# DichenZhang1/libultrahdr_dev

Hardware: AMD Instinct MI355X
Metric: MPixels/sec gain-map generate+apply, 4K P010 batch (higher is better)
Workload: dtype u8/u16 in, f32+f64 math, u8/u32 out

## Files before the change

libultrahdr_dev_amd/build.py:

```python
import os
import subprocess
import sys

HERE = os.path.dirname(os.path.abspath(__file__))
CSRC = os.path.join(HERE, "csrc")
ROOT = os.path.dirname(HERE)
LIB = os.path.join(HERE, "libuhdr_hip.so")
SHIM_LIB = os.path.join(HERE, "libultrahdr_shim.so")
COMM_LIB = os.path.join(HERE, "libuhdr_hip_comm.so")

SOURCES = ["uhdr_kernels.hip", "uhdr_capi.hip", "uhdr_jpeg.hip", "uhdr_jpeg_dec.hip", "uhdr_jpeg_hdr.cpp", "uhdr_jpeg_prog.cpp", "uhdr_jpegr.cpp"]
DEPS = SOURCES + ["uhdr_kernels.h", "uhdr_device_math.h", "uhdr_jpeg.h", "uhdr_jpegr.h", os.path.join(ROOT, "include", "uhdr_hip.h")]
COMM_SOURCES = ["uhdr_comm.hip"]
COMM_DEPS = COMM_SOURCES + [os.path.join(ROOT, "include", "uhdr_hip_comm.h")]
SHIM_SOURCES = ["ultrahdr_shim.cpp"]
SHIM_DEPS = SHIM_SOURCES + [os.path.join(ROOT, "include", "uhdr_hip.h"),
                            os.path.join(ROOT, "include", "ultrahdr_hip", "ultrahdr_hip.h")]

HIPCC = os.environ.get("HIPCC", "/opt/rocm/bin/hipcc")
FLAGS = ["--offload-arch=gfx950", "-O3", "-std=c++17", "-fPIC", "-ffp-contract=off",
         "-fno-fast-math", "-Wall", "-Wno-unused-function"]


def _stale(target, deps, base):
    if not os.path.exists(target):
        return True
    t = os.path.getmtime(target)
    for d in deps:
        p = d if os.path.isabs(d) else os.path.join(base, d)
        if os.path.exists(p) and os.path.getmtime(p) > t:
            return True
    return False


def build(force=False, verbose=False):
    if force or _stale(LIB, DEPS, CSRC):
        cmd = [HIPCC] + FLAGS + ["-shared", "-o", LIB] + [os.path.join(CSRC, s) for s in SOURCES]
        if verbose:
            print(" ".join(cmd))
        subprocess.check_call(cmd)
    shim_src = [os.path.join(CSRC, s) for s in SHIM_SOURCES]
    if all(os.path.exists(s) for s in shim_src) and (force or _stale(SHIM_LIB, SHIM_DEPS, CSRC)):
        cmd = ["g++", "-O2", "-std=c++17", "-fPIC", "-shared", "-I" + os.path.join(ROOT, "include"),
               "-o", SHIM_LIB] + shim_src + ["-L" + HERE, "-luhdr_hip", "-Wl,-rpath,$ORIGIN"]
        if verbose:
            print(" ".join(cmd))
        subprocess.check_call(cmd)
    if force or _stale(COMM_LIB, COMM_DEPS, CSRC):
        rocm_lib = os.path.join(os.path.dirname(os.path.dirname(HIPCC)), "lib")
        cmd = [HIPCC] + FLAGS + ["-shared", "-o", COMM_LIB] + [os.path.join(CSRC, s) for s in COMM_SOURCES] + ["-L" + rocm_lib, "-lrccl", "-Wl,-rpath," + rocm_lib]
        if verbose:
            print(" ".join(cmd))
        try:
            subprocess.check_call(cmd)
        except (subprocess.CalledProcessError, OSError) as e:
            print("libuhdr_hip_comm.so skipped (is RCCL installed under %s?): %s" % (rocm_lib, e), file=sys.stderr)
    return LIB


if __name__ == "__main__":
    print(build(force="--force" in sys.argv, verbose=True))
```

libultrahdr_dev_amd/csrc/uhdr_kernels.hip:

```cpp
#include "uhdr_kernels.h"

#include <hip/hip_runtime.h>

#include <algorithm>
#include <cmath>

#include "uhdr_device_math.h"
#include "uhdr_wave_scan.h"

namespace uhdr {

__constant__ float c_idw4[4 * 64];

__constant__ float c_idw4p[64];

hipError_t upload_idw4(const float* tables) {
  float p[64];
  for (int oy = 0; oy < 4; ++oy)
    for (int pr = 0; pr < 2; ++pr)
      for (int k = 0; k < 4; ++k)
        for (int h = 0; h < 2; ++h) p[((oy * 2 + pr) * 4 + k) * 2 + h] = tables[oy * 16 + (2 * pr + h) * 4 + k];
  hipError_t e = hipMemcpyToSymbol(HIP_SYMBOL(c_idw4p), p, sizeof(p));
  if (e != hipSuccess) return e;
  return hipMemcpyToSymbol(HIP_SYMBOL(c_idw4), tables, sizeof(float) * 4 * 64);
// ... 1272 lines not shown
    o.z = (b * factor) / c.display_boost;
  } else {
    r = srgb_inv_oetf_fast(r); g = srgb_inv_oetf_fast(g); b = srgb_inv_oetf_fast(b);
    const float factor = __builtin_amdgcn_exp2f((log_boost * c.display_boost) * c.inv_max_boost);
    o.x = (r * factor) * c.inv_display_boost;
    o.y = (g * factor) * c.inv_display_boost;
    o.z = (b * factor) * c.inv_display_boost;
  }
  return o;
}

template <int FMT, bool EXACT>
__device__ __forceinline__ F3 hdr_oetf(F3 e) {
  if (FMT == 3) {
    if (EXACT) { float ch[3] = {e.x, e.y, e.z}; hlg_oetf_guarded_n<3>(ch); e.x = ch[0]; e.y = ch[1]; e.z = ch[2]; }
    else { e.x = hlg_oetf_fast(e.x); e.y = hlg_oetf_fast(e.y); e.z = hlg_oetf_fast(e.z); }
  } else if (FMT == 2) {
    if (EXACT) { float ch[3] = {e.x, e.y, e.z}; pq_oetf_guarded_n<3>(ch); e.x = ch[0]; e.y = ch[1]; e.z = ch[2]; }
    else { e.x = pq_oetf_est(e.x); e.y = pq_oetf_est(e.y); e.z = pq_oetf_est(e.z); }
  }
  return e;
}

__device__ __forceinline__ float map_to_float(uint32_t v) { return (float)v / 255.0f; }
__device__ __forceinline__ float map_to_float_fast(uint32_t v) { return div_const((float)v, 255.0f, 1.0f / 255.0f); }

__device__ __forceinline__ f2 log2_2(f2 v) { return (f2){__builtin_amdgcn_logf(v.x), __builtin_amdgcn_logf(v.y)}; }
__device__ __forceinline__ f2 exp2_2(f2 v) { return (f2){__builtin_amdgcn_exp2f(v.x), __builtin_amdgcn_exp2f(v.y)}; }
__device__ __forceinline__ f2 sqrt_2(f2 v) { return (f2){__builtin_amdgcn_sqrtf(v.x), __builtin_amdgcn_sqrtf(v.y)}; }
__device__ __forceinline__ f2 rcp_2(f2 v) { return (f2){__builtin_amdgcn_rcpf(v.x), __builtin_amdgcn_rcpf(v.y)}; }
__device__ __forceinline__ f2 sel_le(f2 x, float thr, f2 a, f2 b) {
  return (f2){x.x <= thr ? a.x : b.x, x.y <= thr ? a.y : b.y};
}


__device__ __forceinline__ f2 srgb_eotf2(f2 e) {
  constexpr float kThr = 0.04045f;
  const f2 a = pk_mul_sat(e, splat(1.0f / kThr));
  const f2 lin = pk_fma(a, splat(kThr / 12.92f), splat(-(kThr / 12.92f)));
  const f2 d = pk_add_sat(e, splat(-kThr));
  const f2 x = pk_fma(d, splat(1.0f / 1.055f), splat((kThr + 0.055f) / 1.055f));
  const f2 t = exp2_2(log2_2(x) * splat(0.4f));
  return pk_fma(x * x, t, lin);
}

__device__ __forceinline__ uint32_t tab_offset(float x) {
  typedef __fp16 h2 __attribute__((ext_vector_type(2)));
  const h2 q = __builtin_amdgcn_cvt_pkrtz(x, 0.0f);
  return __builtin_bit_cast(uint32_t, q) & 0x7FF8u;
}
__device__ __forceinline__ uint32_t pow_offset(float x) {
  uint32_t off;
  asm("v_and_b32_sdwa %0, %1, %2 dst_sel:DWORD dst_unused:UNUSED_PAD src0_sel:DWORD src1_sel:WORD_1" : "=v"(off) : "v"(0x0FF8u), "v"(x));
  return off;
}
__device__ __forceinline__ void pow_pair(f2 x, const char* lut, float2& a, float2& b) {
  a = *reinterpret_cast<const float2*>(lut + pow_offset(x.x));
  b = *reinterpret_cast<const float2*>(lut + pow_offset(x.y));
}
template <uint32_t BASE>
__device__ __forceinline__ void tab_pair(f2 x, const char* lut, float2& a, float2& b) {
  typedef __fp16 h2 __attribute__((ext_vector_type(2)));
  const h2 q = __builtin_amdgcn_cvt_pkrtz(x.x, x.y);
  const uint32_t d = __builtin_bit_cast(uint32_t, q);
  uint32_t hi_off;
  asm("v_and_b32_sdwa %0, %1, %2 dst_sel:DWORD dst_unused:UNUSED_PAD src0_sel:DWORD src1_sel:WORD_1" : "=v"(hi_off) : "v"(0x7FF8u), "v"(d));
  a = *reinterpret_cast<const float2*>(lut + BASE + (d & 0x7FF8u));
  b = *reinterpret_cast<const float2*>(lut + BASE + hi_off);
}
template <uint32_t BASE>
__device__ __forceinline__ f2 tab_eval2(f2 x, const char* lut) {
  float2 a, b;
  tab_pair<BASE>(x, lut, a, b);
  f2 o;
  asm("v_fma_f32 %0, %1, %2, %3" : "=v"(o.x) : "v"(a.y), "v"(x.x), "v"(a.x));
  asm("v_fma_f32 %0, %1, %2, %3" : "=v"(o.y) : "v"(b.y), "v"(x.y), "v"(b.x));
  return o;
}
__device__ __forceinline__ uint32_t s2_address(float s, uint32_t slot8) {
  return __builtin_amdgcn_perm(__float_as_uint(s), slot8, 0x0C0C0600u);
}
__device__ __forceinline__ f2 code_eval2(f2 s, uint32_t slot8, const char* lut) {
  const float2 a = *reinterpret_cast<const float2*>(lut + s2_address(s.x, slot8));
  const float2 b = *reinterpret_cast<const float2*>(lut + s2_address(s.y, slot8));
  f2 o;
  asm("v_fma_f32 %0, %1, %2, %3" : "=v"(o.x) : "v"(a.y), "v"(s.x), "v"(a.x));
  asm("v_fma_f32 %0, %1, %2, %3" : "=v"(o.y) : "v"(b.y), "v"(s.y), "v"(b.x));
  return o;
}

template <int FMT, bool MASK> struct ApplyTab {
  static constexpr bool kOetf = !MASK && (FMT == 2 || FMT == 3);
  static constexpr uint32_t kS1Bytes = kOetf ? kTabS1PowBytes : kTabS1Bytes;
  static constexpr uint32_t kS2Base = kS1Bytes;
  static constexpr uint32_t kS2Bytes = kOetf ? kTabS2LdsBytes : 0u;
  static constexpr uint32_t kBytes = kS1Bytes + kS2Bytes;
  static constexpr uint32_t kS1Float = !kOetf ? kTabS1Lin : FMT == 3 ? kTabS1Hlg : kTabS1Pq;
  static constexpr uint32_t kS2Float = FMT == 3 ? kTabS2Hlg : kTabS2Pq;
};

template <int FMT>
__device__ __forceinline__ f2 oetf2_scaled(f2 e) {
  if (FMT == 3) {
    const f2 lo = sqrt_2(e * splat(3.0f * 1023.0f * 1023.0f));
    const f2 hi = pk_fma(log2_2(pk_fma(e, splat(12.0f), splat(-UHDR_HLG_B))),
                         splat(UHDR_HLG_A * 0.693147180559945f * 1023.0f), splat(UHDR_HLG_C * 1023.0f));
    return sel_le(e, 1.0f / 12.0f, lo, hi);
  } else if (FMT == 2) {
    const f2 p = exp2_2(log2_2(e) * splat(UHDR_PQ_M1));
    const f2 q = pk_fma(p, splat(UHDR_PQ_C2), splat(UHDR_PQ_C1)) * rcp_2(pk_fma(p, splat(UHDR_PQ_C3), splat(1.0f)));
    return exp2_2(pk_fma(log2_2(q), splat(UHDR_PQ_M2), splat(9.99859042974533f)));
  } else if (FMT == 4) {
    return e * splat(1023.0f);
  }
  return e;
}

struct PairOut { f2 r, g, b; };

template <bool MASK>
__device__ __forceinline__ uint32_t pack10_scaled(float r, float g, float b) {
  uint32_t ri = (uint32_t)r, gi = (uint32_t)g, bi = (uint32_t)b;
  if (MASK) { ri &= 0x3ffu; gi &= 0x3ffu; bi &= 0x3ffu; }
  uint32_t t;
  asm("v_lshl_or_b32 %0, %1, 10, %2" : "=v"(t) : "v"(gi), "v"(ri));
  asm("v_lshl_or_b32 %0, %1, 20, %2" : "=v"(t) : "v"(bi), "v"(t));
  return t | 0xC0000000u;
}
__device__ __forceinline__ uint32_t pack10_bits(float r, float g, float b) {
  uint32_t t;
  asm("v_lshl_or_b32 %0, %1, 10, %2" : "=v"(t) : "v"(__float_as_uint(g)), "v"(__float_as_uint(r)));
  asm("v_lshl_or_b32 %0, %1, 20, %2" : "=v"(t) : "v"(__float_as_uint(b)), "v"(t));
  return t;
}

template <int K>
__device__ __forceinline__ float cvt_byte(uint32_t w) { return (float)((w >> (8 * K)) & 0xffu); }

struct PairF { f2 c[3]; f2 factor; float2 e[6]; };
struct PairM { f2 s[3]; float2 e[6]; };
struct ChromaRow { f2 crv, ngs, cbu; };
__device__ __forceinline__ ChromaRow chroma_row(uint32_t uu, uint32_t vv) {
  constexpr float kCrS = kP3Cr * k255, kCbS = kP3Cb * k255, kGCbS = kP3GCb * k255, kGCrS = kP3GCr * k255;
  const f2 uf = (f2){cvt_byte<0>(uu), cvt_byte<1>(uu)};
  const f2 vf = (f2){cvt_byte<0>(vv), cvt_byte<1>(vv)};
  ChromaRow o;
  o.crv = pk_fma(vf, splat(kCrS), splat(-128.0f * kCrS));
  o.cbu = pk_fma(uf, splat(kCbS), splat(-128.0f * kCbS));
  o.ngs = pk_fma(uf, splat(-kGCbS), pk_fma(vf, splat(-kGCrS), splat(128.0f * kGCbS + 128.0f * kGCrS)));
  return o;
}
template <int FMT>
__device__ __forceinline__ void apply_cell_piped(const AppConsts& c, void* dst, uint32_t cx, uint32_t cy,
                                                 const uint32_t (&yrow)[4], const uint32_t (&uu)[2], const uint32_t (&vv)[2],
                                                 float m1, float m2, float m3, float m4, uint32_t slot8, const char* lut) {
  typedef ApplyTab<FMT, false> T;
  ChromaRow cr = chroma_row(uu[0], vv[0]);
  const float a255 = c.fast.A255;
  f2 d23 = (f2){m2 - m1, m3 - m1}, d4b = (f2){m4 - m1, __builtin_fmaf(m1, a255, c.fast.B)};
  asm("" : "+v"(d23), "+v"(d4b));
  PairF pf[2];
  PairM pm[2];
  uint32_t px[4];
#pragma unroll
  for (int k = 0; k < 10; ++k) {
    if (k < 8) {
      const int oy = k >> 1, pr = k & 1;
      const f2 w1 = (f2){c.fast.wD[oy][pr][0][0], c.fast.wD[oy][pr][0][1]}, w2 = (f2){c.fast.wD[oy][pr][1][0], c.fast.wD[oy][pr][1][1]};
      const f2 w3 = (f2){c.fast.wD[oy][pr][2][0], c.fast.wD[oy][pr][2][1]};
      if (k == 4) cr = chroma_row(uu[1], vv[1]);
      PairF& f = pf[k & 1];
      const f2 E = pk_fma(bc_lo(d4b), w3, pk_fma(bc_hi(d23), w2, pk_fma(bc_lo(d23), w1, bc_hi(d4b))));
      const f2 yraw = pr ? (f2){cvt_byte<2>(yrow[oy]), cvt_byte<3>(yrow[oy])} : (f2){cvt_byte<0>(yrow[oy]), cvt_byte<1>(yrow[oy])};
      if (pr) {
        f.c[0] = pk_fma_sat_bc<1>(yraw, splat(k255), cr.crv); f.c[1] = pk_fma_sat_bc<1>(yraw, splat(k255), cr.ngs);
        f.c[2] = pk_fma_sat_bc<1>(yraw, splat(k255), cr.cbu);
      } else {
        f.c[0] = pk_fma_sat_bc<0>(yraw, splat(k255), cr.crv); f.c[1] = pk_fma_sat_bc<0>(yraw, splat(k255), cr.ngs);
        f.c[2] = pk_fma_sat_bc<0>(yraw, splat(k255), cr.cbu);
      }
      f.factor = exp2_2(E);
#pragma unroll
      for (int ch = 0; ch < 3; ++ch) pow_pair(f.c[ch], lut, f.e[2 * ch], f.e[2 * ch + 1]);
    }
    __builtin_amdgcn_sched_barrier(0);
    if (k >= 1 && k <= 8) {
      PairF& f = pf[(k - 1) & 1];
      PairM& m = pm[(k - 1) & 1];
#pragma unroll
      for (int ch = 0; ch < 3; ++ch) {
        f2 t;
        asm("v_fma_f32 %0, %1, %2, %3" : "=v"(t.x) : "v"(f.e[2 * ch].y), "v"(f.c[ch].x), "v"(f.e[2 * ch].x));
        asm("v_fma_f32 %0, %1, %2, %3" : "=v"(t.y) : "v"(f.e[2 * ch + 1].y), "v"(f.c[ch].y), "v"(f.e[2 * ch + 1].x));
        m.s[ch] = pk_fma(t, f.factor, splat(2.0f));
      }
#pragma unroll
      for (int ch = 0; ch < 3; ++ch) {
        m.e[2 * ch] = *reinterpret_cast<const float2*>(lut + T::kS2Base + s2_address(m.s[ch].x, slot8));
        m.e[2 * ch + 1] = *reinterpret_cast<const float2*>(lut + T::kS2Base + s2_address(m.s[ch].y, slot8));
      }
    }
    __builtin_amdgcn_sched_barrier(0);
    if (k >= 2) {
      const int q = k - 2, oy = q >> 1, pr = q & 1;
      PairM& m = pm[q & 1];
      float o[6];
#pragma unroll
      for (int ch = 0; ch < 3; ++ch) {
        asm("v_fma_f32 %0, %1, %2, %3" : "=v"(o[2 * ch]) : "v"(m.e[2 * ch].y), "v"(m.s[ch].x), "v"(m.e[2 * ch].x));
        asm("v_fma_f32 %0, %1, %2, %3" : "=v"(o[2 * ch + 1]) : "v"(m.e[2 * ch + 1].y), "v"(m.s[ch].y), "v"(m.e[2 * ch + 1].x));
      }
      px[2 * pr] = pack10_bits(o[0], o[2], o[4]);
      px[2 * pr + 1] = pack10_bits(o[1], o[3], o[5]);
      if (pr) {
        const uint32_t off = ((4u * cy + oy) * c.width + 4u * cx) * 4u;
        st_stream(reinterpret_cast<uint4*>(static_cast<char*>(dst) + off), make_uint4(px[0], px[1], px[2], px[3]));
      }
    }
    __builtin_amdgcn_sched_barrier(0);
  }
}

constexpr uint32_t kXchSecond = 72;
constexpr uint32_t kXchPerWave = 136;
template <int FMT, bool MASK>
__device__ __forceinline__ void apply_cell_piped1(const AppConsts& c, const AppImage& im, uint32_t cx, uint32_t cy,
                                                  const uint32_t (&yrow)[4], const uint32_t (&uu)[2], const uint32_t (&vv)[2],
                                                  float m1, float m2, float m3, float m4, const char* lut, uint4* xch) {
  ChromaRow cr = chroma_row(uu[0], vv[0]);
  const float a255 = c.fast.A255;
  f2 d23 = (f2){m2 - m1, m3 - m1}, d4b = (f2){m4 - m1, __builtin_fmaf(m1, a255, c.fast.B)};
  asm("" : "+v"(d23), "+v"(d4b));
  PairF pf[2];
  PairOut po[2];
  const uint32_t lane = threadIdx.x & 63u;
#pragma unroll
  for (int k = 0; k < 9; ++k) {
    if (k < 8) {
      const int oy = k >> 1, pr = k & 1;
      const f2 w1 = (f2){c.fast.wD[oy][pr][0][0], c.fast.wD[oy][pr][0][1]}, w2 = (f2){c.fast.wD[oy][pr][1][0], c.fast.wD[oy][pr][1][1]};
      const f2 w3 = (f2){c.fast.wD[oy][pr][2][0], c.fast.wD[oy][pr][2][1]};
      if (k == 4) cr = chroma_row(uu[1], vv[1]);
      PairF& f = pf[k & 1];
      const f2 E = pk_fma(bc_lo(d4b), w3, pk_fma(bc_hi(d23), w2, pk_fma(bc_lo(d23), w1, bc_hi(d4b))));
      const f2 yraw = pr ? (f2){cvt_byte<2>(yrow[oy]), cvt_byte<3>(yrow[oy])} : (f2){cvt_byte<0>(yrow[oy]), cvt_byte<1>(yrow[oy])};
      if (pr) {
        f.c[0] = pk_fma_sat_bc<1>(yraw, splat(k255), cr.crv); f.c[1] = pk_fma_sat_bc<1>(yraw, splat(k255), cr.ngs);
        f.c[2] = pk_fma_sat_bc<1>(yraw, splat(k255), cr.cbu);
      } else {
        f.c[0] = pk_fma_sat_bc<0>(yraw, splat(k255), cr.crv); f.c[1] = pk_fma_sat_bc<0>(yraw, splat(k255), cr.ngs);
        f.c[2] = pk_fma_sat_bc<0>(yraw, splat(k255), cr.cbu);
      }
      f.factor = exp2_2(E);
#pragma unroll
      for (int ch = 0; ch < 3; ++ch) tab_pair<0>(f.c[ch], lut, f.e[2 * ch], f.e[2 * ch + 1]);
    }
    __builtin_amdgcn_sched_barrier(0);
    if (k >= 1) {
      const int q = k - 1, oy = q >> 1, pr = q & 1;
      PairF& f = pf[q & 1];
      f2 lin[3];
#pragma unroll
      for (int ch = 0; ch < 3; ++ch) {
        f2 t;
        asm("v_fma_f32 %0, %1, %2, %3" : "=v"(t.x) : "v"(f.e[2 * ch].y), "v"(f.c[ch].x), "v"(f.e[2 * ch].x));
        asm("v_fma_f32 %0, %1, %2, %3" : "=v"(t.y) : "v"(f.e[2 * ch + 1].y), "v"(f.c[ch].y), "v"(f.e[2 * ch + 1].x));
        lin[ch] = oetf2_scaled<FMT>(t * f.factor);
      }
      po[pr].r = lin[0]; po[pr].g = lin[1]; po[pr].b = lin[2];
      if (pr) {
        const uint32_t pix0 = (4u * cy + oy) * c.width + 4u * cx;
        if (FMT == 2 || FMT == 3) {
          uint4 o;
          o.x = pack10_scaled<MASK>(po[0].r.x, po[0].g.x, po[0].b.x); o.y = pack10_scaled<MASK>(po[0].r.y, po[0].g.y, po[0].b.y);
          o.z = pack10_scaled<MASK>(po[1].r.x, po[1].g.x, po[1].b.x); o.w = pack10_scaled<MASK>(po[1].r.y, po[1].g.y, po[1].b.y);
          st_stream(reinterpret_cast<uint4*>(static_cast<uint32_t*>(im.dst) + pix0), o);
        } else if (FMT == 1) {
          const uint2 a = pack_f16_hw(po[0].r.x, po[0].g.x, po[0].b.x), bb = pack_f16_hw(po[0].r.y, po[0].g.y, po[0].b.y);
          const uint2 cc = pack_f16_hw(po[1].r.x, po[1].g.x, po[1].b.x), d = pack_f16_hw(po[1].r.y, po[1].g.y, po[1].b.y);
          if (xch != nullptr) {
            xch[lane] = make_uint4(a.x, a.y, bb.x, bb.y);
            xch[kXchSecond + lane] = make_uint4(cc.x, cc.y, d.x, d.y);
            __builtin_amdgcn_wave_barrier();
            const uint32_t from = (lane & 1u) * kXchSecond + (lane >> 1);
            const uint4 s0 = xch[from], s1 = xch[from + 32u];
            __builtin_amdgcn_wave_barrier();
            uint4* o = reinterpret_cast<uint4*>(static_cast<uint2*>(im.dst) + (uint32_t)__builtin_amdgcn_readfirstlane((int)pix0));
            st_stream(o + lane, s0);
            st_stream(o + 64u + lane, s1);
          } else {
            uint4* o = reinterpret_cast<uint4*>(static_cast<uint2*>(im.dst) + pix0);
            o[0] = make_uint4(a.x, a.y, bb.x, bb.y);
            o[1] = make_uint4(cc.x, cc.y, d.x, d.y);
          }
        } else {
          const size_t plane = (size_t)c.width * c.height;
          uint16_t* base16 = static_cast<uint16_t*>(im.dst);
          const f2 ch[3][2] = {{po[0].r, po[1].r}, {po[0].g, po[1].g}, {po[0].b, po[1].b}};
#pragma unroll
          for (int p = 0; p < 3; ++p) {
            const uint32_t q0 = 0x3ffu & (uint32_t)ch[p][0].x, q1 = 0x3ffu & (uint32_t)ch[p][0].y;
            const uint32_t q2 = 0x3ffu & (uint32_t)ch[p][1].x, q3 = 0x3ffu & (uint32_t)ch[p][1].y;
            st_stream(reinterpret_cast<uint2*>(base16 + p * plane + pix0), make_uint2(q0 | (q1 << 16), q2 | (q3 << 16)));
          }
        }
      }
    }
    __builtin_amdgcn_sched_barrier(0);
  }
}

struct ApplyCellIn { uint32_t yrow[4], uu[2], vv[2], mb[4]; };
__device__ __forceinline__ void apply_load_cell(const AppConsts& c, const AppImage& im, uint32_t cx, uint32_t cy, ApplyCellIn& o) {
  const uint32_t yoff = 4u * cy * im.y_stride + 4u * cx;
#pragma unroll
  for (int r = 0; r < 4; ++r) o.yrow[r] = ld_stream(reinterpret_cast<const uint32_t*>(im.y + (yoff + r * im.y_stride)));
  const uint32_t coff = 2u * cy * im.c_stride + 2u * cx;
#pragma unroll
  for (int r = 0; r < 2; ++r) {
    o.uu[r] = *reinterpret_cast<const uint16_t*>(im.u + (coff + r * im.c_stride));
    o.vv[r] = *reinterpret_cast<const uint16_t*>(im.v + (coff + r * im.c_stride));
  }
  const uint32_t xu = min(cx + 1u, c.map_w - 1u), yu = min(cy + 1u, c.map_h - 1u);
  const uint32_t m0 = cy * c.map_w, m1 = yu * c.map_w;
  o.mb[0] = im.map[m0 + cx]; o.mb[1] = im.map[m1 + cx]; o.mb[2] = im.map[m0 + xu]; o.mb[3] = im.map[m1 + xu];
}

template <int FMT, bool MASK>
__device__ __forceinline__ void apply_cell_edge(const AppConsts& c, const AppImage& im, uint32_t cx, uint32_t cy,
                                                const uint32_t (&yrow)[4], const uint32_t (&uu)[2], const uint32_t (&vv)[2],
                                                float m1, float m2, float m3, float m4, const float* wt ,
                                                uint32_t slot8, const char* lut) {
  typedef ApplyTab<FMT, MASK> T;
  const float a255 = c.fast.A255;
  const float base = __builtin_fmaf(m1, a255, c.fast.B), d2 = m2 - m1, d3 = m3 - m1, d4 = m4 - m1;
#pragma unroll 1
  for (uint32_t oy = 0; oy < 4u; ++oy) {
    const uint32_t yw = oy == 0u ? yrow[0] : oy == 1u ? yrow[1] : oy == 2u ? yrow[2] : yrow[3];
    const ChromaRow cr = chroma_row(oy < 2u ? uu[0] : uu[1], oy < 2u ? vv[0] : vv[1]);
    const uint32_t pix0 = (4u * cy + oy) * c.width + 4u * cx;
    uint32_t px[4];
    PairOut po[2];
#pragma unroll
    for (int pr = 0; pr < 2; ++pr) {
      const f2 yraw = pr ? (f2){cvt_byte<2>(yw), cvt_byte<3>(yw)} : (f2){cvt_byte<0>(yw), cvt_byte<1>(yw)};
      const float* p0 = wt + oy * 16u + pr * 8;
      const f2 w1 = (f2){p0[1], p0[5]}, w2 = (f2){p0[2], p0[6]}, w3 = (f2){p0[3], p0[7]};
      const f2 E = pk_fma(splat(d4), w3, pk_fma(splat(d3), w2, pk_fma(splat(d2), w1, splat(base))));
      const f2 factor = exp2_2(E);
      f2 ch[3];
      if (pr) {
        ch[0] = pk_fma_sat_bc<1>(yraw, splat(k255), cr.crv); ch[1] = pk_fma_sat_bc<1>(yraw, splat(k255), cr.ngs); ch[2] = pk_fma_sat_bc<1>(yraw, splat(k255), cr.cbu);
      } else {
        ch[0] = pk_fma_sat_bc<0>(yraw, splat(k255), cr.crv); ch[1] = pk_fma_sat_bc<0>(yraw, splat(k255), cr.ngs); ch[2] = pk_fma_sat_bc<0>(yraw, splat(k255), cr.cbu);
      }
      if (T::kOetf) {
        float o[6];
#pragma unroll
        for (int q = 0; q < 3; ++q) {
          float2 a, b;
          pow_pair(ch[q], lut, a, b);
          f2 t;
          asm("v_fma_f32 %0, %1, %2, %3" : "=v"(t.x) : "v"(a.y), "v"(ch[q].x), "v"(a.x));
          asm("v_fma_f32 %0, %1, %2, %3" : "=v"(t.y) : "v"(b.y), "v"(ch[q].y), "v"(b.x));
          const f2 s = pk_fma(t, factor, splat(2.0f));
          const float2 ea = *reinterpret_cast<const float2*>(lut + T::kS2Base + s2_address(s.x, slot8));
          const float2 eb = *reinterpret_cast<const float2*>(lut + T::kS2Base + s2_address(s.y, slot8));
          asm("v_fma_f32 %0, %1, %2, %3" : "=v"(o[2 * q]) : "v"(ea.y), "v"(s.x), "v"(ea.x));
          asm("v_fma_f32 %0, %1, %2, %3" : "=v"(o[2 * q + 1]) : "v"(eb.y), "v"(s.y), "v"(eb.x));
        }
        px[2 * pr] = pack10_bits(o[0], o[2], o[4]);
        px[2 * pr + 1] = pack10_bits(o[1], o[3], o[5]);
      } else {
        f2 lin[3];
#pragma unroll
        for (int q = 0; q < 3; ++q) {
          float2 a, b;
          tab_pair<0>(ch[q], lut, a, b);
          f2 t;
          asm("v_fma_f32 %0, %1, %2, %3" : "=v"(t.x) : "v"(a.y), "v"(ch[q].x), "v"(a.x));
          asm("v_fma_f32 %0, %1, %2, %3" : "=v"(t.y) : "v"(b.y), "v"(ch[q].y), "v"(b.x));
          lin[q] = oetf2_scaled<FMT>(t * factor);
        }
        po[pr].r = lin[0]; po[pr].g = lin[1]; po[pr].b = lin[2];
      }
    }
    if (T::kOetf) {
      st_stream(reinterpret_cast<uint4*>(static_cast<uint32_t*>(im.dst) + pix0), make_uint4(px[0], px[1], px[2], px[3]));
    } else if (FMT == 2 || FMT == 3) {
      uint4 o;
      o.x = pack10_scaled<MASK>(po[0].r.x, po[0].g.x, po[0].b.x); o.y = pack10_scaled<MASK>(po[0].r.y, po[0].g.y, po[0].b.y);
      o.z = pack10_scaled<MASK>(po[1].r.x, po[1].g.x, po[1].b.x); o.w = pack10_scaled<MASK>(po[1].r.y, po[1].g.y, po[1].b.y);
      st_stream(reinterpret_cast<uint4*>(static_cast<uint32_t*>(im.dst) + pix0), o);
    } else if (FMT == 1) {
      const uint2 a = pack_f16_hw(po[0].r.x, po[0].g.x, po[0].b.x), bb = pack_f16_hw(po[0].r.y, po[0].g.y, po[0].b.y);
      const uint2 cc = pack_f16_hw(po[1].r.x, po[1].g.x, po[1].b.x), d = pack_f16_hw(po[1].r.y, po[1].g.y, po[1].b.y);
      uint4* o = reinterpret_cast<uint4*>(static_cast<uint2*>(im.dst) + pix0);
      o[0] = make_uint4(a.x, a.y, bb.x, bb.y);
      o[1] = make_uint4(cc.x, cc.y, d.x, d.y);
    } else {
      const size_t plane = (size_t)c.width * c.height;
      uint16_t* base16 = static_cast<uint16_t*>(im.dst);
      const f2 pl[3][2] = {{po[0].r, po[1].r}, {po[0].g, po[1].g}, {po[0].b, po[1].b}};
#pragma unroll
      for (int p = 0; p < 3; ++p) {
        const uint32_t q0 = 0x3ffu & (uint32_t)pl[p][0].x, q1 = 0x3ffu & (uint32_t)pl[p][0].y;
        const uint32_t q2 = 0x3ffu & (uint32_t)pl[p][1].x, q3 = 0x3ffu & (uint32_t)pl[p][1].y;
        st_stream(reinterpret_cast<uint2*>(base16 + p * plane + pix0), make_uint2(q0 | (q1 << 16), q2 | (q3 << 16)));
      }
    }
  }
}

struct ApplyCellPk { uint32_t yrow[4], uu[2], vv[2], mrow[2]; };
struct __attribute__((packed)) U16Any { uint16_t v; };
__device__ __forceinline__ void apply_load_cell_pk(const AppConsts& c, const AppImage& im, uint32_t cx, uint32_t cy, uint32_t mx, uint32_t cy1, ApplyCellPk& o) {
  const uint32_t yoff = 4u * cy * im.y_stride + 4u * cx;
#pragma unroll
  for (int r = 0; r < 4; ++r) o.yrow[r] = ld_stream(reinterpret_cast<const uint32_t*>(im.y + (yoff + r * im.y_stride)));
  const uint32_t coff = 2u * cy * im.c_stride + 2u * cx;
#pragma unroll
  for (int r = 0; r < 2; ++r) {
    o.uu[r] = *reinterpret_cast<const uint16_t*>(im.u + (coff + r * im.c_stride));
    o.vv[r] = *reinterpret_cast<const uint16_t*>(im.v + (coff + r * im.c_stride));
  }
  o.mrow[0] = reinterpret_cast<const U16Any*>(im.map + (cy * c.map_w + mx))->v;
  o.mrow[1] = reinterpret_cast<const U16Any*>(im.map + (cy1 * c.map_w + mx))->v;
}

constexpr uint32_t kApplyBlock = 512;
constexpr uint32_t kApplyMaxCellsPerThread = 32;

template <int FMT, bool MASK>
__device__ __forceinline__ bool apply_walk_cell(const AppConsts& c, const AppImage& im, uint32_t& cx, uint32_t& cy, uint32_t& left,
                                                const ApplyCellPk& cur, ApplyCellPk& nxt, uint32_t slot8, const char* lut,
                                                const float* s_idw, uint4* s_xch) {
  typedef ApplyTab<FMT, MASK> T;
  uint32_t ncx = cx + c.step_x, ncy = cy + c.step_y;
  if (ncx >= c.map_w) { ncx -= c.map_w; ++ncy; }
  --left;
  const bool more = left != 0u && ncy < c.map_h;
  if (!more) { ncx = cx; ncy = cy; }
  apply_load_cell_pk(c, im, ncx, ncy, ncx - (ncx + 1u == c.map_w ? 1u : 0u), min(ncy + 1u, c.map_h - 1u), nxt);
  const bool edge_x = cx + 1u == c.map_w, edge_y = cy + 1u == c.map_h;
  const float e3 = cvt_byte<1>(cur.mrow[0]), e4 = cvt_byte<1>(cur.mrow[1]);
  const float e1 = edge_x ? e3 : cvt_byte<0>(cur.mrow[0]), e2 = edge_x ? e4 : cvt_byte<0>(cur.mrow[1]);
  const bool interior = __builtin_amdgcn_ballot_w64(edge_x || edge_y) == 0ull;
  const float* wt = s_idw + (edge_x ? (edge_y ? 192 : 64) : (edge_y ? 128 : 0));
  if (T::kOetf) {
    if (interior) apply_cell_piped<FMT>(c, im.dst, cx, cy, cur.yrow, cur.uu, cur.vv, e1, e2, e3, e4, slot8, lut);
    else apply_cell_edge<FMT, MASK>(c, im, cx, cy, cur.yrow, cur.uu, cur.vv, e1, e2, e3, e4, wt, slot8, lut);
  } else {
    uint4* xch = nullptr;
    if (FMT == 1 && __builtin_amdgcn_ballot_w64(true) == ~0ull &&
        __builtin_amdgcn_ballot_w64(cy != (uint32_t)__builtin_amdgcn_readfirstlane((int)cy)) == 0ull)
      xch = s_xch + (threadIdx.x >> 6) * kXchPerWave;
    if (interior) apply_cell_piped1<FMT, MASK>(c, im, cx, cy, cur.yrow, cur.uu, cur.vv, e1, e2, e3, e4, lut, xch);
    else apply_cell_edge<FMT, MASK>(c, im, cx, cy, cur.yrow, cur.uu, cur.vv, e1, e2, e3, e4, wt, slot8, lut);
  }
  cx = ncx; cy = ncy;
  return more;
}

template <int FMT, bool MASK>
__global__ void __launch_bounds__(kApplyBlock, 4) k_apply_s4(const AppConsts c, const AppBatch b) {
  typedef ApplyTab<FMT, MASK> T;
  __shared__ uint4 s_tab[T::kBytes / 16u];
  __shared__ uint4 s_xch[FMT == 1 ? (kApplyBlock / 64) * kXchPerWave : 1];
  __shared__ float s_idw[4 * 64];
  const uint32_t img_i = blockIdx.x, span = blockIdx.y;
  const AppImage& im = b.img[img_i];
  const uint32_t idx = span * c.cells_per_thread * kApplyBlock + threadIdx.x;
  uint32_t cy = idx / c.map_w;
  uint32_t cx = idx - cy * c.map_w;
  const bool any = cy < c.map_h;
  ApplyCellPk ca, cb;
  if (any) apply_load_cell_pk(c, im, cx, cy, cx - (cx + 1u == c.map_w ? 1u : 0u), min(cy + 1u, c.map_h - 1u), ca);
  {
    constexpr uint32_t kN1 = T::kS1Bytes / 16u, kPer1 = (kN1 + kApplyBlock - 1u) / kApplyBlock;
    constexpr uint32_t kN2 = T::kOetf ? kTabS2Cells * 32u : 0u, kPer2 = (kN2 + kApplyBlock - 1u) / kApplyBlock;
    const uint4* src1 = reinterpret_cast<const uint4*>(c.tab + T::kS1Float);
    const uint2* src2 = reinterpret_cast<const uint2*>(c.tab + T::kS2Float);
    uint4 t1[kPer1];
    uint2 t2[kPer2 ? kPer2 : 1u];
    const float w = c_idw4[threadIdx.x & 255u] * c.fast.A255;
#pragma unroll
    for (uint32_t k = 0; k < kPer1; ++k) { const uint32_t i = k * kApplyBlock + threadIdx.x; t1[k] = src1[i < kN1 ? i : kN1 - 1u]; }
#pragma unroll
    for (uint32_t k = 0; k < kPer2; ++k) { const uint32_t i = k * kApplyBlock + threadIdx.x; t2[k] = src2[(i < kN2 ? i : 0u) >> 5]; }
    if (threadIdx.x < 256u) s_idw[threadIdx.x] = w;
#pragma unroll
    for (uint32_t k = 0; k < kPer1; ++k) { const uint32_t i = k * kApplyBlock + threadIdx.x; if (i < kN1) s_tab[i] = t1[k]; }
#pragma unroll
    for (uint32_t k = 0; k < kPer2; ++k) { const uint32_t i = k * kApplyBlock + threadIdx.x; if (i < kN2) reinterpret_cast<uint2*>(s_tab)[T::kS2Base / 8u + i] = t2[k]; }
  }
  __syncthreads();
  const char* lut = reinterpret_cast<const char*>(s_tab);
  const uint32_t slot8 = (threadIdx.x & 31u) << 3;
  if (!any) return;
  if (T::kOetf) {
    asm volatile("s_setreg_imm32_b32 hwreg(HW_REG_MODE, 0, 2), 3" : "+v"(cx), "+v"(cy));
  }
  uint32_t left = c.cells_per_thread;
#pragma unroll 1
  for (;;) {
    if (!apply_walk_cell<FMT, MASK>(c, im, cx, cy, left, ca, cb, slot8, lut, s_idw, s_xch)) return;
    if (!apply_walk_cell<FMT, MASK>(c, im, cx, cy, left, cb, ca, slot8, lut, s_idw, s_xch)) return;
  }
}

struct PxIn { float yf, u, v, gain; };
struct PxTaps { uint32_t xl, xu, yl, yu; const float* w; };
__device__ __forceinline__ PxTaps px_taps(const AppConsts& c, uint32_t x, uint32_t y);
__device__ __forceinline__ PxIn px_inputs(const AppConsts& c, const AppImage& im, uint32_t x, uint32_t y) {
  PxIn in;
  in.yf = (float)im.y[(size_t)y * im.y_stride + x] * k255;
  const size_t ci = (size_t)(y >> im.csy) * im.c_stride + (x >> im.csx);
  in.u = (float)((int)im.u[ci] - 128) * k255;
  in.v = (float)((int)im.v[ci] - 128) * k255;
  const PxTaps t = px_taps(c, x, y);
  const float e1 = map_to_float_fast(im.map[(size_t)t.yl * c.map_w + t.xl]);
  const float e2 = map_to_float_fast(im.map[(size_t)t.yu * c.map_w + t.xl]);
  const float e3 = map_to_float_fast(im.map[(size_t)t.yl * c.map_w + t.xu]);
  const float e4 = map_to_float_fast(im.map[(size_t)t.yu * c.map_w + t.xu]);
  in.gain = e1 * t.w[0] + e2 * t.w[1] + e3 * t.w[2] + e4 * t.w[3];
  return in;
}
__device__ __forceinline__ PxTaps px_taps(const AppConsts& c, uint32_t x, uint32_t y) {
  const uint32_t s = c.scale;
  uint32_t xl, yl, ox, oy;
  if ((s & (s - 1u)) == 0u) {
    const uint32_t sh = (uint32_t)__builtin_ctz(s);
    xl = x >> sh; yl = y >> sh; ox = x & (s - 1u); oy = y & (s - 1u);
  } else {
    xl = x / s; yl = y / s; ox = x - xl * s; oy = y - yl * s;
  }
  uint32_t xu = xl + 1u, yu = yl + 1u;
  xl = min(xl, c.map_w - 1u); xu = min(xu, c.map_w - 1u);
  yl = min(yl, c.map_h - 1u); yu = min(yu, c.map_h - 1u);
  int tbl = 0;
  if (xl == xu && yl == yu) tbl = 3;
  else if (xl == xu) tbl = 1;
  else if (yl == yu) tbl = 2;
  PxTaps t;
  t.xl = xl; t.xu = xu; t.yl = yl; t.yu = yu;
  t.w = c.idw + (size_t)tbl * s * s * 4u + (size_t)oy * s * 4u + ox * 4u;
  return t;
}
__host__ __device__ inline dim3 px_grid(uint32_t width, uint32_t height, int n) {
  return dim3((width + 255u) / 256u, height < 65535u ? height : 65535u, (unsigned)n);
}
template <int FMT>
__device__ __forceinline__ void px_store(const AppImage& im, size_t idx, size_t total, F3 e) {
  if (FMT == 2 || FMT == 3) {
    static_cast<uint32_t*>(im.dst)[idx] = pack_1010102(e.x, e.y, e.z);
  } else if (FMT == 1) {
    static_cast<uint2*>(im.dst)[idx] = pack_f16(e.x, e.y, e.z);
  } else {
    uint16_t* base = static_cast<uint16_t*>(im.dst);
    base[idx] = (uint16_t)(0x3ffu & (uint32_t)(e.x * 1023.0f));
    base[total + idx] = (uint16_t)(0x3ffu & (uint32_t)(e.y * 1023.0f));
    base[2 * total + idx] = (uint16_t)(0x3ffu & (uint32_t)(e.z * 1023.0f));
  }
}

template <int FMT, bool EXACT>
__global__ void __launch_bounds__(256) k_apply_px(const AppConsts c, const AppBatch b) {
  const AppImage& im = b.img[blockIdx.z];
  const size_t total = (size_t)c.width * c.height;
  const uint32_t x = blockIdx.x * 256u + threadIdx.x;
  if (x >= c.width) return;
  for (uint32_t y = blockIdx.y; y < c.height; y += gridDim.y) {
    const PxIn in = px_inputs(c, im, x, y);
    const F3 lin = recover_hdr<EXACT>(c, in.yf, kP3Cr * in.v, kP3GCb * in.u, kP3GCr * in.v, kP3Cb * in.u, in.gain);
    px_store<FMT>(im, (size_t)y * c.width + x, total, hdr_oetf<FMT, EXACT>(lin));
  }
}

template <bool EXACT>
__device__ __forceinline__ F3 recover_hdr_rgb(const AppConsts& c, float yf, float crv, float gcbu, float gcrv, float cbu,
                                              const float (&gain)[3]) {
  float ch[3] = {clamp01(yf + crv), clamp01(yf - gcbu - gcrv), clamp01(yf + cbu)};
  float o[3];
  if (EXACT) srgb_inv_oetf_guarded_n<3>(ch);
#pragma unroll
  for (int k = 0; k < 3; ++k) {
    const float log_boost = (float)(c.log2_min_d * (double)(1.0f - gain[k]) + c.log2_max_d * (double)gain[k]);
    if (EXACT) {
      const float factor = exp2_to_float_guarded(log_boost * c.display_boost / c.max_boost);
      o[k] = (ch[k] * factor) / c.display_boost;
    } else {
      const float factor = __builtin_amdgcn_exp2f((log_boost * c.display_boost) * c.inv_max_boost);
      o[k] = (srgb_inv_oetf_fast(ch[k]) * factor) * c.inv_display_boost;
    }
  }
  F3 r;
  r.x = o[0]; r.y = o[1]; r.z = o[2];
  return r;
}
template <int FMT, bool EXACT>
__global__ void __launch_bounds__(256) k_apply_px_rgb(const AppConsts c, const AppBatch b) {
  const AppImage& im = b.img[blockIdx.z];
  const uint32_t* map = reinterpret_cast<const uint32_t*>(im.map);
  const size_t total = (size_t)c.width * c.height;
  const uint32_t x = blockIdx.x * 256u + threadIdx.x;
  if (x >= c.width) return;
  for (uint32_t y = blockIdx.y; y < c.height; y += gridDim.y) {
    const float yf = (float)im.y[(size_t)y * im.y_stride + x] * k255;
    const size_t ci = (size_t)(y >> im.csy) * im.c_stride + (x >> im.csx);
    const float u = (float)((int)im.u[ci] - 128) * k255, v = (float)((int)im.v[ci] - 128) * k255;
    const PxTaps t = px_taps(c, x, y);
    const uint32_t m1 = map[(size_t)t.yl * c.map_stride + t.xl], m2 = map[(size_t)t.yu * c.map_stride + t.xl];
    const uint32_t m3 = map[(size_t)t.yl * c.map_stride + t.xu], m4 = map[(size_t)t.yu * c.map_stride + t.xu];
    const float w0 = t.w[0], w1 = t.w[1], w2 = t.w[2], w3 = t.w[3];
    float gain[3];
#pragma unroll
    for (int k = 0; k < 3; ++k)
      gain[k] = map_to_float_fast((m1 >> (8 * k)) & 0xffu) * w0 + map_to_float_fast((m2 >> (8 * k)) & 0xffu) * w1 +
                map_to_float_fast((m3 >> (8 * k)) & 0xffu) * w2 + map_to_float_fast((m4 >> (8 * k)) & 0xffu) * w3;
    const F3 lin = recover_hdr_rgb<EXACT>(c, yf, kP3Cr * v, kP3GCb * u, kP3GCr * v, kP3Cb * u, gain);
    px_store<FMT>(im, (size_t)y * c.width + x, total, hdr_oetf<FMT, EXACT>(lin));
  }
}
template <int FMT>
static hipError_t launch_apply_rgb_t(const AppConsts& c, const AppBatch& b, int n, bool exact, hipStream_t s) {
  if (n == 0 || c.width == 0 || c.height == 0) return hipSuccess;
  const dim3 grid = px_grid(c.width, c.height, n);
  if (exact) hipLaunchKernelGGL((k_apply_px_rgb<FMT, true>), grid, dim3(256), 0, s, c, b);
  else hipLaunchKernelGGL((k_apply_px_rgb<FMT, false>), grid, dim3(256), 0, s, c, b);
  return hipGetLastError();
}
hipError_t launch_apply_rgb(const AppConsts& c, const AppBatch& b, int n, int fmt, bool exact, hipStream_t s) {
  switch (fmt) {
    case 1: return launch_apply_rgb_t<1>(c, b, n, exact, s);
    case 2: return launch_apply_rgb_t<2>(c, b, n, exact, s);
    case 3: return launch_apply_rgb_t<3>(c, b, n, exact, s);
    case 4: return launch_apply_rgb_t<4>(c, b, n, exact, s);
    default: return hipErrorInvalidValue;
  }
}

template <bool GAMMA>
__device__ __forceinline__ float md_factor(const AppMdConsts& m, float g) {
  if (GAMMA) g = __builtin_amdgcn_exp2f(__builtin_amdgcn_logf(g) * m.inv_gamma);
  return __builtin_amdgcn_exp2f(__builtin_fmaf(g, m.A, m.B));
}
__device__ __forceinline__ float md_channel(const AppMdConsts& m, float e, float factor) {
// ... 1748 lines not shown
```

Measured before the change: 547,600.

## Shrink apply cell chroma fields, buffer edge-cell stores, make walk loop wave-uniform

Several changes land together in the apply kernel. The chroma and map fields in the per-cell struct shrink to 16 bits, which cuts register pressure. Edge-cell outputs are buffered for all four rows and written after the row loop instead of inside it. The loop-continue condition becomes wave-uniform through a ballot, and the LDS exchange path is chosen by a boolean that also checks the lanes hold contiguous cx. A compiler flag lets structurization skip uniform regions, and asm sinks keep the table-preload registers live; together these aim at control-flow and register costs. The shrunk uu/vv fields feed cvt_byte, which reads bytes 0 and 1, so that stays valid if the values fit in 16 bits. Buffering edge rows adds register use, and the ballot-based loop runs lanes that have finished on redundant work.

```diff
diff --git a/libultrahdr_dev_amd/build.py b/libultrahdr_dev_amd/build.py
--- a/libultrahdr_dev_amd/build.py
+++ b/libultrahdr_dev_amd/build.py
@@ -20,6 +20,7 @@
 HIPCC = os.environ.get("HIPCC", "/opt/rocm/bin/hipcc")
 FLAGS = ["--offload-arch=gfx950", "-O3", "-std=c++17", "-fPIC", "-ffp-contract=off",
          "-fno-fast-math", "-Wall", "-Wno-unused-function"]
+FLAGS += ["-mllvm", "-structurizecfg-skip-uniform-regions"]
 
 
 def _stale(target, deps, base):
diff --git a/libultrahdr_dev_amd/csrc/uhdr_kernels.hip b/libultrahdr_dev_amd/csrc/uhdr_kernels.hip
--- a/libultrahdr_dev_amd/csrc/uhdr_kernels.hip
+++ b/libultrahdr_dev_amd/csrc/uhdr_kernels.hip
@@ -1448,7 +1448,7 @@
 }
 template <int FMT>
 __device__ __forceinline__ void apply_cell_piped(const AppConsts& c, void* dst, uint32_t cx, uint32_t cy,
-                                                 const uint32_t (&yrow)[4], const uint32_t (&uu)[2], const uint32_t (&vv)[2],
+                                                 const uint32_t (&yrow)[4], const uint16_t (&uu)[2], const uint16_t (&vv)[2],
                                                  float m1, float m2, float m3, float m4, uint32_t slot8, const char* lut) {
   typedef ApplyTab<FMT, false> T;
   ChromaRow cr = chroma_row(uu[0], vv[0]);
@@ -1521,8 +1521,9 @@
 constexpr uint32_t kXchPerWave = 136;
 template <int FMT, bool MASK>
 __device__ __forceinline__ void apply_cell_piped1(const AppConsts& c, const AppImage& im, uint32_t cx, uint32_t cy,
-                                                  const uint32_t (&yrow)[4], const uint32_t (&uu)[2], const uint32_t (&vv)[2],
-                                                  float m1, float m2, float m3, float m4, const char* lut, uint4* xch) {
+                                                  const uint32_t (&yrow)[4], const uint16_t (&uu)[2], const uint16_t (&vv)[2],
+                                                  float m1, float m2, float m3, float m4, const char* lut, uint4* xch,
+                                                  bool via_xch ) {
   ChromaRow cr = chroma_row(uu[0], vv[0]);
   const float a255 = c.fast.A255;
   f2 d23 = (f2){m2 - m1, m3 - m1}, d4b = (f2){m4 - m1, __builtin_fmaf(m1, a255, c.fast.B)};
@@ -1574,7 +1575,7 @@
         } else if (FMT == 1) {
           const uint2 a = pack_f16_hw(po[0].r.x, po[0].g.x, po[0].b.x), bb = pack_f16_hw(po[0].r.y, po[0].g.y, po[0].b.y);
           const uint2 cc = pack_f16_hw(po[1].r.x, po[1].g.x, po[1].b.x), d = pack_f16_hw(po[1].r.y, po[1].g.y, po[1].b.y);
-          if (xch != nullptr) {
+          if (via_xch) {
             xch[lane] = make_uint4(a.x, a.y, bb.x, bb.y);
             xch[kXchSecond + lane] = make_uint4(cc.x, cc.y, d.x, d.y);
             __builtin_amdgcn_wave_barrier();
@@ -1624,18 +1625,24 @@
 
 template <int FMT, bool MASK>
 __device__ __forceinline__ void apply_cell_edge(const AppConsts& c, const AppImage& im, uint32_t cx, uint32_t cy,
-                                                const uint32_t (&yrow)[4], const uint32_t (&uu)[2], const uint32_t (&vv)[2],
+                                                const uint32_t (&yrow)[4], const uint16_t (&uu)[2], const uint16_t (&vv)[2],
                                                 float m1, float m2, float m3, float m4, const float* wt ,
                                                 uint32_t slot8, const char* lut) {
   typedef ApplyTab<FMT, MASK> T;
   const float a255 = c.fast.A255;
   const float base = __builtin_fmaf(m1, a255, c.fast.B), d2 = m2 - m1, d3 = m3 - m1, d4 = m4 - m1;
+  constexpr int kW = FMT == 4 ? 3 : FMT == 1 ? 2 : 1;
+  uint4 rows[4][kW];
+#pragma unroll
+  for (int r = 0; r < 4; ++r)
+#pragma unroll
+    for (int q = 0; q < kW; ++q) rows[r][q] = make_uint4(0u, 0u, 0u, 0u);
 #pragma unroll 1
   for (uint32_t oy = 0; oy < 4u; ++oy) {
     const uint32_t yw = oy == 0u ? yrow[0] : oy == 1u ? yrow[1] : oy == 2u ? yrow[2] : yrow[3];
     const ChromaRow cr = chroma_row(oy < 2u ? uu[0] : uu[1], oy < 2u ? vv[0] : vv[1]);
-    const uint32_t pix0 = (4u * cy + oy) * c.width + 4u * cx;
     uint32_t px[4];
+    uint4 row[kW];
     PairOut po[2];
 #pragma unroll
     for (int pr = 0; pr < 2; ++pr) {
@@ -1682,33 +1689,48 @@
       }
     }
     if (T::kOetf) {
-      st_stream(reinterpret_cast<uint4*>(static_cast<uint32_t*>(im.dst) + pix0), make_uint4(px[0], px[1], px[2], px[3]));
+      row[0] = make_uint4(px[0], px[1], px[2], px[3]);
     } else if (FMT == 2 || FMT == 3) {
-      uint4 o;
-      o.x = pack10_scaled<MASK>(po[0].r.x, po[0].g.x, po[0].b.x); o.y = pack10_scaled<MASK>(po[0].r.y, po[0].g.y, po[0].b.y);
-      o.z = pack10_scaled<MASK>(po[1].r.x, po[1].g.x, po[1].b.x); o.w = pack10_scaled<MASK>(po[1].r.y, po[1].g.y, po[1].b.y);
-      st_stream(reinterpret_cast<uint4*>(static_cast<uint32_t*>(im.dst) + pix0), o);
+      row[0].x = pack10_scaled<MASK>(po[0].r.x, po[0].g.x, po[0].b.x); row[0].y = pack10_scaled<MASK>(po[0].r.y, po[0].g.y, po[0].b.y);
+      row[0].z = pack10_scaled<MASK>(po[1].r.x, po[1].g.x, po[1].b.x); row[0].w = pack10_scaled<MASK>(po[1].r.y, po[1].g.y, po[1].b.y);
     } else if (FMT == 1) {
       const uint2 a = pack_f16_hw(po[0].r.x, po[0].g.x, po[0].b.x), bb = pack_f16_hw(po[0].r.y, po[0].g.y, po[0].b.y);
       const uint2 cc = pack_f16_hw(po[1].r.x, po[1].g.x, po[1].b.x), d = pack_f16_hw(po[1].r.y, po[1].g.y, po[1].b.y);
-      uint4* o = reinterpret_cast<uint4*>(static_cast<uint2*>(im.dst) + pix0);
-      o[0] = make_uint4(a.x, a.y, bb.x, bb.y);
-      o[1] = make_uint4(cc.x, cc.y, d.x, d.y);
+      row[0] = make_uint4(a.x, a.y, bb.x, bb.y);
+      row[kW - 1] = make_uint4(cc.x, cc.y, d.x, d.y);
     } else {
-      const size_t plane = (size_t)c.width * c.height;
-      uint16_t* base16 = static_cast<uint16_t*>(im.dst);
       const f2 pl[3][2] = {{po[0].r, po[1].r}, {po[0].g, po[1].g}, {po[0].b, po[1].b}};
 #pragma unroll
       for (int p = 0; p < 3; ++p) {
         const uint32_t q0 = 0x3ffu & (uint32_t)pl[p][0].x, q1 = 0x3ffu & (uint32_t)pl[p][0].y;
         const uint32_t q2 = 0x3ffu & (uint32_t)pl[p][1].x, q3 = 0x3ffu & (uint32_t)pl[p][1].y;
-        st_stream(reinterpret_cast<uint2*>(base16 + p * plane + pix0), make_uint2(q0 | (q1 << 16), q2 | (q3 << 16)));
-      }
-    }
-  }
-}
-
-struct ApplyCellPk { uint32_t yrow[4], uu[2], vv[2], mrow[2]; };
+        row[p % kW] = make_uint4(q0 | (q1 << 16), q2 | (q3 << 16), 0u, 0u);
+      }
+    }
+#pragma unroll
+    for (int q = 0; q < kW; ++q) { rows[0][q] = rows[1][q]; rows[1][q] = rows[2][q]; rows[2][q] = rows[3][q]; rows[3][q] = row[q]; }
+  }
+  char* const dst = static_cast<char*>(im.dst);
+  const uint32_t pix0 = 4u * cy * c.width + 4u * cx;
+#pragma unroll
+  for (uint32_t oy = 0; oy < 4u; ++oy) {
+    const uint32_t pix = pix0 + oy * c.width;
+    if (FMT == 2 || FMT == 3) {
+      st_stream(reinterpret_cast<uint4*>(dst + pix * 4u), rows[oy][0]);
+    } else if (FMT == 1) {
+      uint4* o = reinterpret_cast<uint4*>(dst + pix * 8u);
+      o[0] = rows[oy][0];
+      o[1] = rows[oy][kW - 1];
+    } else {
+      const uint32_t plane2 = c.width * c.height * 2u;
+#pragma unroll
+      for (int p = 0; p < 3; ++p)
+        st_stream(reinterpret_cast<uint2*>(dst + (p * plane2 + pix * 2u)), make_uint2(rows[oy][p % kW].x, rows[oy][p % kW].y));
+    }
+  }
+}
+
+struct ApplyCellPk { uint32_t yrow[4]; uint16_t uu[2], vv[2], mrow[2]; };
 struct __attribute__((packed)) U16Any { uint16_t v; };
 __device__ __forceinline__ void apply_load_cell_pk(const AppConsts& c, const AppImage& im, uint32_t cx, uint32_t cy, uint32_t mx, uint32_t cy1, ApplyCellPk& o) {
   const uint32_t yoff = 4u * cy * im.y_stride + 4u * cx;
@@ -1735,8 +1757,9 @@
   uint32_t ncx = cx + c.step_x, ncy = cy + c.step_y;
   if (ncx >= c.map_w) { ncx -= c.map_w; ++ncy; }
   --left;
-  const bool more = left != 0u && ncy < c.map_h;
-  if (!more) { ncx = cx; ncy = cy; }
+  const bool mine = left != 0u && ncy < c.map_h;
+  const bool more = __builtin_amdgcn_ballot_w64(mine) != 0ull;
+  if (!mine) { ncx = cx; ncy = cy; }
   apply_load_cell_pk(c, im, ncx, ncy, ncx - (ncx + 1u == c.map_w ? 1u : 0u), min(ncy + 1u, c.map_h - 1u), nxt);
   const bool edge_x = cx + 1u == c.map_w, edge_y = cy + 1u == c.map_h;
   const float e3 = cvt_byte<1>(cur.mrow[0]), e4 = cvt_byte<1>(cur.mrow[1]);
@@ -1747,11 +1770,11 @@
     if (interior) apply_cell_piped<FMT>(c, im.dst, cx, cy, cur.yrow, cur.uu, cur.vv, e1, e2, e3, e4, slot8, lut);
     else apply_cell_edge<FMT, MASK>(c, im, cx, cy, cur.yrow, cur.uu, cur.vv, e1, e2, e3, e4, wt, slot8, lut);
   } else {
-    uint4* xch = nullptr;
-    if (FMT == 1 && __builtin_amdgcn_ballot_w64(true) == ~0ull &&
-        __builtin_amdgcn_ballot_w64(cy != (uint32_t)__builtin_amdgcn_readfirstlane((int)cy)) == 0ull)
-      xch = s_xch + (threadIdx.x >> 6) * kXchPerWave;
-    if (interior) apply_cell_piped1<FMT, MASK>(c, im, cx, cy, cur.yrow, cur.uu, cur.vv, e1, e2, e3, e4, lut, xch);
+    uint4* const xch = s_xch + (FMT == 1 ? (threadIdx.x >> 6) * kXchPerWave : 0u);
+    const bool via_xch = FMT == 1 && __builtin_amdgcn_ballot_w64(true) == ~0ull &&
+        __builtin_amdgcn_ballot_w64(cy != (uint32_t)__builtin_amdgcn_readfirstlane((int)cy) ||
+                                    cx != (uint32_t)__builtin_amdgcn_readfirstlane((int)cx) + (threadIdx.x & 63u)) == 0ull;
+    if (interior) apply_cell_piped1<FMT, MASK>(c, im, cx, cy, cur.yrow, cur.uu, cur.vv, e1, e2, e3, e4, lut, xch, via_xch);
     else apply_cell_edge<FMT, MASK>(c, im, cx, cy, cur.yrow, cur.uu, cur.vv, e1, e2, e3, e4, wt, slot8, lut);
   }
   cx = ncx; cy = ncy;
@@ -1789,6 +1812,10 @@
     for (uint32_t k = 0; k < kPer1; ++k) { const uint32_t i = k * kApplyBlock + threadIdx.x; if (i < kN1) s_tab[i] = t1[k]; }
 #pragma unroll
     for (uint32_t k = 0; k < kPer2; ++k) { const uint32_t i = k * kApplyBlock + threadIdx.x; if (i < kN2) reinterpret_cast<uint2*>(s_tab)[T::kS2Base / 8u + i] = t2[k]; }
+#pragma unroll
+    for (uint32_t k = 0; k < kPer1; ++k) asm volatile("" :: "v"(t1[k].w));
+#pragma unroll
+    for (uint32_t k = 0; k < kPer2; ++k) asm volatile("" :: "v"(t2[k].y));
   }
   __syncthreads();
   const char* lut = reinterpret_cast<const char*>(s_tab);
```

Result: faster. 555,400, median of 6 (+1.4%).
